# prashantpandeygit/solvingpapers

Measured on AMD Instinct MI355X. Metric: training tokens/sec, LLaMA3-8B-shape bf16, higher is better.
Workload: dtype bf16; 1 GPU; model=llama3_8b, global_batch=4, seq_len=8192, parallelism=dp1, micro_batch=1, grad_accum=4, params=8030261248

## Files before the change

### csrc/include/attn_params.h

```cpp
#pragma once
#include "attn_common.h"

#define SPA_DBG_BRH(b, r, R, h, H) (SPA_DBG_OK(b, p.B) & SPA_DBG_OK(r, R) & SPA_DBG_OK(h, H))

namespace spa {

struct AttnParams {
  const bf16* q; const bf16* k; const bf16* v; const bf16* o; const bf16* dout;
  bf16* out; bf16* dq; bf16* dk; bf16* dv;
  float* lse; const float* lse_in; float* delta; float* dqacc;
  int B, H, Hkv, Tq, Tk;
  long sqb, sqt, sqh, skb, skt, skh, svb, svt, svh, sob, sot, soh;
  long sdob, sdot, sdoh;
  long sdqb, sdqt, sdqh, sdkb, sdkt, sdkh, sdvb, sdvt, sdvh;
  float scale;
  float scale_log2;
  int causal_off;
  int hsplit;
  float* dkacc; float* dvacc;
  unsigned seed_lo, seed_hi, drop_thr;
  float drop_scale;
  const int64_t* seed_ptr;
  long long* stamp;
  int xcd;
  bf16* dsbuf;
  long ds_kvstride;
  int ds_nqt, ds_nkt;
  int ksplit;
  float* part;
  float* mlpart;
  int part_ld;
  int vhalf;
  float* rowk;
  int rowk_ld;
};

void launch_dkdv5(AttnParams& p, bool causal, hipStream_t st);
void launch_bwd_short(AttnParams& p, bool causal, hipStream_t st);

__device__ __forceinline__ long ds_index(int qt, int kt, int g, int G, int nkt, bool causal) {
  const int qb = qt >> 1, t = qt & 1;
  const long step = causal ? (long)qb * (qb + 1) + kt : (long)qb * nkt + kt;
  return (step * G + g) * 2 + t;
}
inline long ds_kv_elems(int nq64, int nkt, int G, bool causal) {
  return 1024L * 2 * G * (causal ? (long)nq64 * (nq64 + 1) : (long)nq64 * nkt);
}
__device__ __forceinline__ int ds_slot(int s, int h, int k) { return (k >> 2) * 16 + (2 * s + h) * 4 + (k & 3); }

template <int HD, int NDT = HD / 32>
__device__ __forceinline__ void store_kv_grad(const AttnParams& p, const f32x16 (&acc)[NDT], bool is_k,
                                              int b, int hk, int key, int split, int hh, int dt0 = 0) {
  if (key >= p.Tk) return;
  if (!(SPA_DBG_BRH(b, key, p.Tk, hk, p.Hkv) & SPA_DBG_OK(split, p.hsplit))) return;
  static_assert(NDT <= HD / 32, "store_kv_grad: more tiles than the head dim");
  constexpr int DT = NDT;
  if (p.hsplit == 1) {
    bf16* dst = (is_k ? p.dk + b * p.sdkb + (long)key * p.sdkt + hk * p.sdkh
                      : p.dv + b * p.sdvb + (long)key * p.sdvt + hk * p.sdvh) + 32 * dt0;
    const float sc = is_k ? p.scale : 1.f;
#pragma unroll
    for (int dt = 0; dt < DT; ++dt)
#pragma unroll
      for (int g = 0; g < 4; ++g) {
        bf16x4 w;
#pragma unroll
        for (int i = 0; i < 4; ++i) w[i] = (bf16)(acc[dt][4 * g + i] * sc);
        *reinterpret_cast<bf16x4*>(dst + 32 * dt + 8 * g + 4 * hh) = w;
      }
  } else {
    float* dst = (is_k ? p.dkacc : p.dvacc) +
                 ((((long)split * p.B + b) * p.Tk + key) * p.Hkv + hk) * HD + 32 * dt0;
#pragma unroll
    for (int dt = 0; dt < DT; ++dt)
#pragma unroll
      for (int g = 0; g < 4; ++g) {
        f32x4 w;
#pragma unroll
        for (int i = 0; i < 4; ++i) w[i] = acc[dt][4 * g + i];
        *reinterpret_cast<f32x4*>(dst + 32 * dt + 8 * g + 4 * hh) = w;
      }
  }
// ... 5 lines not shown
```

### csrc/kernels/attention.hip

```cpp
#include "attn_common.h"
#include "attn_params.h"

SPA_DEBUG_TU("attention.hip")

namespace spa {



__device__ __forceinline__ unsigned mix32(unsigned x) {
  x ^= x >> 16; x *= 0x7feb352dU; x ^= x >> 15; x *= 0x846ca68bU; x ^= x >> 16;
  return x;
}
__device__ __forceinline__ unsigned drop_base(const AttnParams& p, int b, int h) {
  unsigned lo = p.seed_lo, hi = p.seed_hi;
  if (p.seed_ptr) {
    const uint64_t sd = (uint64_t)*p.seed_ptr;
    lo = (unsigned)(sd & 0xffffffffu);
    hi = (unsigned)(sd >> 32);
  }
  return mix32(lo ^ mix32(hi + (unsigned)(b * p.H + h) * 0x9E3779B9U));
}
__device__ __forceinline__ bool drop_keep(unsigned base, int q, int key, unsigned thr) {
  return (mix32(base + (unsigned)q * 0x85EBCA6BU + (unsigned)key * 0xC2B2AE35U) >> 8) >= thr;
}
// ... 15 lines not shown
  } else {
    const int nbh = p.H * p.B;
    const int bh = bi % nbh;
    qb = bi / nbh;
    if (causal) qb = nqb - 1 - qb;
    h = bh % p.H;
    b = bh / p.H;
  }
}

template <int HDK, int HDV> constexpr int attn_bn() { return (HDK >= 256 || HDV >= 256) ? 32 : 64; }

#ifndef FWD_PV_SCHED
#define FWD_PV_SCHED 1
#endif
template <int HDK, int HDV, int NW, bool CAUSAL, bool DROP>
__global__ __launch_bounds__(NW * 64) void attn_fwd_kernel(AttnParams p) {
  constexpr int BN = attn_bn<HDK, HDV>(), NSUB = BN / 32, BM = 32 * NW, KS = HDK / 16, DT = HDV / 32;
  constexpr int NT = NW * 64, IK = img_w<HDK>(), IV = img_w<HDV>();
  constexpr int TK = BN * IK, TV = BN * IV, TB = TK + TV;
  __shared__ __attribute__((aligned(16))) bf16 smem[2 * TB];
  const int tid = threadIdx.x, lane = tid & 63, wave = tid >> 6;
  const int lq = lane & 31, hh = lane >> 5;
  const int nqb = cdiv(p.Tq, BM);
  const int si = blockIdx.x % p.ksplit;
  int qb, b, h;
  q_block_map(p, nqb, CAUSAL, qb, b, h, blockIdx.x / p.ksplit, gridDim.x / p.ksplit);
  const int hk = h / (p.H / p.Hkv);
  SPA_DBG_CHECK(qb, nqb);
  SPA_DBG_CHECK(hk, p.Hkv);
  (void)SPA_DBG_BRH(b, 0, 1, h, p.H);
  const int q0 = __builtin_amdgcn_readfirstlane(qb * BM + wave * 32);
  const int q = q0 + lq;
  const float c = p.scale_log2;
  const int vcol = blockIdx.y * p.vhalf;
  unsigned dbase = 0;
  if constexpr (DROP) dbase = drop_base(p, b, h);

  bf16x8 qf[KS];
  {
    const bf16* qp = p.q + b * p.sqb + (long)q * p.sqt + h * p.sqh + 8 * hh;
#pragma unroll
    for (int s = 0; s < KS; ++s) qf[s] = q < p.Tq ? *reinterpret_cast<const bf16x8*>(qp + 16 * s) : zero8();
  }
  f32x16 o[DT];
#pragma unroll
  for (int i = 0; i < DT; ++i) o[i] = splat16(0.f);
  float m = -1e30f, l = 0.f;

  int kend = p.Tk;
  if (CAUSAL) kend = min(p.Tk, qb * BM + BM + p.causal_off);
  const int wave_kend = q0 >= p.Tq ? 0 : CAUSAL ? min(p.Tk, q0 + 32 + p.causal_off) : p.Tk;
  const int ntiles_all = kend > 0 ? cdiv(kend, BN) : 0;
  const int kper = cdiv(ntiles_all, p.ksplit);
  const int jbeg = min(ntiles_all, si * kper);
  const int ntiles = min(ntiles_all, jbeg + kper) - jbeg;
  const int kb0 = jbeg * BN;

// ... 1108 lines not shown
      store_kv_grad<HDV>(p, av, false, b, hk, key, split, hh);
    }
  }
#if SPA_DKDV3_STAMP
  DK3_TICK(4);
  if (p.stamp != nullptr && lane < 8) {
    long long v = 0;
#pragma unroll
    for (int i = 0; i < 5; ++i) v = lane == i ? seg[i] : v;
    v = lane == 5 ? (long long)(total + 1) : lane == 6 ? ts_ - t_start : v;
    p.stamp[((long)blockIdx.x * 8 + wave) * 8 + lane] = v;
  }
#endif
}

template <int HD, bool CAUSAL, bool NT>
__global__ __launch_bounds__(256, 2) void attn_bwd_dq_ds_kernel(AttnParams p) {
  static_assert(HD == 128, "dq_ds: head dim 128 (K tile = 4 KiB-row images of 256 B)");
  constexpr int DT = HD / 32, KIMG = 32 * HD, WSLOT = 2 * 1024, SLOT = KIMG + 4 * WSLOT, NSLOT = 3;
  __shared__ __attribute__((aligned(16))) bf16 smem[NSLOT * SLOT];
  const int tid = threadIdx.x, lane = tid & 63;
  const int wave = __builtin_amdgcn_readfirstlane(tid >> 6);
  const int hh = lane >> 5;
  const int G = p.H / p.Hkv;
  const int nq64 = cdiv(p.Tq, 64);
  const int upkv = nq64 * G;
  const int wgpkv = cdiv(upkv, 4);
  const int nbkv = p.B * p.Hkv;
  const int bkv = blockIdx.x % nbkv;
  const int w = CAUSAL ? wgpkv - 1 - (int)(blockIdx.x / nbkv) : (int)(blockIdx.x / nbkv);
  const int b = bkv / p.Hkv, hk = bkv % p.Hkv;
// ... 84 lines not shown
        if (jj + 1 < nsteps) asm volatile("s_waitcnt vmcnt(6)" ::: "memory");
        else asm volatile("s_waitcnt vmcnt(0)" ::: "memory");
        asm volatile("s_waitcnt lgkmcnt(0)" ::: "memory");
        __builtin_amdgcn_s_barrier();
        if (jj + 2 < nsteps) issue(jj + 2, (r + 2) % 3);
        compute(jj, smem + r * SLOT);
      }
    }
  }
  if (!uvalid) return;
#pragma unroll
  for (int t = 0; t < 2; ++t) {
    const int q = qb * 64 + 32 * t + (lane & 31);
    if (q >= p.Tq || !SPA_DBG_BRH(b, q, p.Tq, h, p.H)) continue;
    bf16* op = p.dq + b * p.sdqb + (long)q * p.sdqt + h * p.sdqh;
#pragma unroll
    for (int dt = 0; dt < DT; ++dt)
#pragma unroll
      for (int g = 0; g < 4; ++g) {
        bf16x4 wv;
#pragma unroll
        for (int i = 0; i < 4; ++i) wv[i] = (bf16)(acc[t][dt][4 * g + i] * p.scale);
        *reinterpret_cast<bf16x4*>(op + 32 * dt + 8 * g + 4 * hh) = wv;
      }
  }
}

template <int HDK, bool CAUSAL, bool NT>
__global__ __launch_bounds__(256, 2) void attn_bwd_dq_ds256_kernel(AttnParams p) {
  static_assert(HDK == 256 || HDK == 192, "dq_ds256: q/k head dim 192 or 256");
  constexpr int HD = 256, DT = HDK / 32, KIMG = 32 * HD, WSLOT = 1024, SLOT = KIMG + 4 * WSLOT, NSLOT = 3;
  __shared__ __attribute__((aligned(16))) bf16 smem[NSLOT * SLOT];
  const int tid = threadIdx.x, lane = tid & 63;
  const int wave = __builtin_amdgcn_readfirstlane(tid >> 6);
  const int hh = lane >> 5;
  const int G = p.H / p.Hkv;
  const int nqt = cdiv(p.Tq, 32);
  const int upkv = nqt * G;
  const int wgpkv = cdiv(upkv, 4);
// ... 296 lines not shown
  TORCH_CHECK(dropout_p >= 0.0 && dropout_p < 1.0, "attention dropout p must be in [0, 1)");
  p.seed_lo = (unsigned)(seed & 0xffffffffu);
  p.seed_hi = (unsigned)(((uint64_t)seed >> 32) & 0xffffffffu);
  p.drop_thr = (unsigned)std::llround(dropout_p * 16777216.0);
  p.drop_scale = (float)(1.0 / (1.0 - dropout_p));
}

static int attn_ksplit(long blocks, int ntk) {
  const char* e = getenv("SPA_ATTN_KSPLIT");
  if (e) return std::max(1, std::min(atoi(e), std::max(1, ntk)));
  int ks = 1;
  while (blocks * ks < 512 && ks < 8 && ntk / (2 * ks) >= 4) ks *= 2;
  return ks;
}

std::vector<at::Tensor> attn_fwd(const at::Tensor& q, const at::Tensor& k, const at::Tensor& v, double scale,
                                 bool causal, double dropout_p, int64_t seed,
                                 const c10::optional<at::Tensor>& seed_t) {
  check_qkv(q, "q"); check_qkv(k, "k"); check_qkv(v, "v");
  const int B = q.size(0), Tq = q.size(1), H = q.size(2), HDK = q.size(3), HDV = v.size(3);
  const int Tk = k.size(1), Hkv = k.size(2);
  TORCH_CHECK(k.size(0) == B && v.size(0) == B && v.size(1) == Tk && v.size(2) == Hkv && k.size(3) == HDK,
              "attn: shape mismatch");
  TORCH_CHECK(H % Hkv == 0, "attn: H must be a multiple of Hkv");
  const bool drop = dropout_p > 0.0;
  TORCH_CHECK(!drop || HDK == HDV, "attn: dropout needs equal q/k and v head dims");
  DeviceGuard g(q.device());
  auto out = at::empty({B, Tq, H, HDV}, q.options());
  auto lse = at::empty({B, H, Tq}, q.options().dtype(at::kFloat));
  AttnParams p{};
  p.q = (const bf16*)q.data_ptr(); p.k = (const bf16*)k.data_ptr(); p.v = (const bf16*)v.data_ptr();
  p.out = (bf16*)out.data_ptr(); p.lse = lse.data_ptr<float>();
  p.B = B; p.H = H; p.Hkv = Hkv; p.Tq = Tq; p.Tk = Tk;
  fill_strides(p, q, k, v);
  fill_dropout(p, dropout_p, seed, seed_t);
  p.sob = out.stride(0); p.sot = out.stride(1); p.soh = out.stride(2);
  p.scale = (float)scale; p.scale_log2 = (float)(scale * 1.4426950408889634);
  p.causal_off = Tk - Tq;
  p.hsplit = 1;
  p.ksplit = 1;
  p.xcd = xcd_order(B, Hkv);
  if (B * Tq * H == 0) return {out, lse};
  auto st = stream();
  const char* f2e = getenv("SPA_ATTN_FWD256");
  const bool pshare = !(f2e && atoi(f2e) == 0) && HDK == 256 && HDV == 256 && !drop;
  const char* sve = getenv("SPA_ATTN_SPLITV");
  const bool splitv = !pshare && !(sve && atoi(sve) == 0) && HDK == 256 && HDV == 256 && !drop;
  const int nw = splitv || pshare ? 8 : (HDK <= 192 && HDV <= 192) || (HDK == 256 && HDV == 128) ? 8 : 4;
  const int blocks = cdiv(Tq, pshare ? 128 : 32 * nw) * H * B * (splitv ? 2 : 1);
  const int ntk = cdiv(Tk, (HDK >= 256 || HDV >= 256) ? 32 : 64);
  p.ksplit = attn_ksplit(blocks, ntk);
  at::Tensor part;
  if (p.ksplit > 1) {
    const long rows = (long)B * H * Tq;
    part = at::empty({(long)p.ksplit * rows * (HDV + 2)}, q.options().dtype(at::kFloat));
    p.part = part.data_ptr<float>();
    p.part_ld = HDV;
    p.mlpart = p.part + (long)p.ksplit * rows * HDV;
  }
  const int gx = blocks / (splitv ? 2 : 1) * p.ksplit;
  if (pshare) {
    if (causal) attn_fwd256p_kernel<true><<<gx, 512, 0, st>>>(p);
    else attn_fwd256p_kernel<false><<<gx, 512, 0, st>>>(p);
  } else if (splitv) {
    p.vhalf = 128;
    if (causal) attn_fwd_kernel<256, 128, 8, true, false><<<dim3(gx, 2), 512, 0, st>>>(p);
    else attn_fwd_kernel<256, 128, 8, false, false><<<dim3(gx, 2), 512, 0, st>>>(p);
  } else {
    HDKV_SWITCH(HDK, HDV, {
      constexpr int NW = fwd_waves<HDK_, HDV_>();
      constexpr bool SQ = HDK_ == HDV_;
      if (drop) {
        if constexpr (SQ) {
          if (causal) attn_fwd_kernel<HDK_, HDV_, NW, true, true><<<gx, NW * 64, 0, st>>>(p);
          else attn_fwd_kernel<HDK_, HDV_, NW, false, true><<<gx, NW * 64, 0, st>>>(p);
        }
      } else {
        if (causal) attn_fwd_kernel<HDK_, HDV_, NW, true, false><<<gx, NW * 64, 0, st>>>(p);
        else attn_fwd_kernel<HDK_, HDV_, NW, false, false><<<gx, NW * 64, 0, st>>>(p);
      }
    });
  }
  if (p.ksplit > 1) {
    const long n = (long)B * H * Tq * (HDV / 8);
    HDKV_SWITCH(HDK, HDV, { attn_fwd_merge_kernel<HDV_><<<(int)cdiv(n, 256L), 256, 0, st>>>(p); });
  }
  SPA_LAUNCH_CHECK();
  return {out, lse};
}

template <int HDK, int HDV, bool DROP>
static void launch_bwd(AttnParams& p, bool causal, bool fused, int dkdv_mode, int nkv, hipStream_t st,
                       const at::TensorOptions& bf16_opts) {
// ... 9 lines not shown
      else attn_bwd_dkdv_kernel<HDK, HDV, false, MT, true, false><<<g2, 256, 0, st>>>(p);
      const long n = rows * (HDK / 8);
      attn_dq_store_kernel<HDK><<<(int)std::min<long>((n + 255) / 256, 65536), 256, 0, st>>>(p);
      return;
    }
  }
  if constexpr (HDK == 128 && HDV == 128 && !DROP) {
    const char* de = getenv("SPA_ATTN_DQ_DS");
    const bool want = !(de && atoi(de) == 0);
    const long kv_bytes = 2 * ds_kv_elems(cdiv(p.Tq, 64), cdiv(p.Tk, 32), p.H / p.Hkv, causal);
    if (want && p.hsplit == 1 && p.Tk > 0 && dkdv_mode == 0 && (!causal || p.causal_off == 0) &&
        kv_bytes < 0x7fffffffL) {
      const long rows = (long)p.B * p.Tq * p.H;
      const char* v5e = getenv("SPA_ATTN_DKDV5");
      const bool v5 = !(v5e && atoi(v5e) == 0);
      if (!v5) attn_delta_kernel<HDK><<<(int)cdiv(rows, 256 / (HDK / 8)), 256, 0, st>>>(p);
      p.ds_nqt = cdiv(p.Tq, 32);
      p.ds_nkt = cdiv(p.Tk, 32);
      p.ds_kvstride = ds_kv_elems(cdiv(p.Tq, 64), p.ds_nkt, p.H / p.Hkv, causal);
      at::Tensor dsb = at::empty({(long)p.B * p.Hkv * p.ds_kvstride}, bf16_opts);
      p.dsbuf = (bf16*)dsb.data_ptr();
      at::Tensor rowk;
      if (v5) {
        p.rowk_ld = cdiv(p.Tq, 64) * 64;
        rowk = at::empty({(long)p.B * p.H * 2 * p.rowk_ld}, bf16_opts.dtype(at::kFloat));
        p.rowk = rowk.data_ptr<float>();
        launch_dkdv5(p, causal, st);
      } else if (causal) attn_bwd_dkdv3_kernel<HDK, HDV, true, true><<<nkv, 512, 0, st>>>(p);
      else attn_bwd_dkdv3_kernel<HDK, HDV, false, true><<<nkv, 512, 0, st>>>(p);
      const int G = p.H / p.Hkv;
      const int wg = cdiv(cdiv(p.Tq, 64) * G, 4) * p.B * p.Hkv;
      const char* ne = getenv("SPA_ATTN_DS_NT");
      const bool nt = !(ne && atoi(ne) == 0);
      if (nt) {
        if (causal) attn_bwd_dq_ds_kernel<HDK, true, true><<<wg, 256, 0, st>>>(p);
        else attn_bwd_dq_ds_kernel<HDK, false, true><<<wg, 256, 0, st>>>(p);
      } else {
        if (causal) attn_bwd_dq_ds_kernel<HDK, true, false><<<wg, 256, 0, st>>>(p);
        else attn_bwd_dq_ds_kernel<HDK, false, false><<<wg, 256, 0, st>>>(p);
      }
      return;
    }
  }
  if constexpr (((HDK == 256 && HDV == 256) || (HDK == 192 && HDV == 128)) && !DROP) {
    const char* de = getenv("SPA_ATTN_DQ_DS");
    const int dsm = de ? atoi(de) : 1;
    const bool want = dsm != 0;
    const int G = p.H / p.Hkv;
    const long kv_bytes = 2 * ds_kv_elems(cdiv(p.Tq, 64), cdiv(p.Tk, 32), G, causal);
// ... 90 lines not shown
    const long rows = (long)p.B * p.Tk * p.Hkv;
    attn_kv_reduce_kernel<HDK><<<(int)std::min<long>((rows * (HDK / 8) + 255) / 256, 65536), 256, 0, st>>>(p, 1);
    attn_kv_reduce_kernel<HDV><<<(int)std::min<long>((rows * (HDV / 8) + 255) / 256, 65536), 256, 0, st>>>(p, 0);
  }
}

static at::Tensor& last_stamps() {
  static at::Tensor t;
  return t;
}
at::Tensor attn_bwd_stamps() { return last_stamps().defined() ? last_stamps().view({-1, 8}).clone() : at::Tensor(); }

void attn_bwd(const at::Tensor& dout, const at::Tensor& q, const at::Tensor& k, const at::Tensor& v,
              const at::Tensor& out, const at::Tensor& lse, const at::Tensor& dq, const at::Tensor& dk,
              const at::Tensor& dv, double scale, bool causal, double dropout_p, int64_t seed,
              const c10::optional<at::Tensor>& seed_t) {
  check_qkv(dout, "dout"); check_qkv(q, "q"); check_qkv(k, "k"); check_qkv(v, "v"); check_qkv(out, "out");
  check_qkv(dq, "dq"); check_qkv(dk, "dk"); check_qkv(dv, "dv");
  const int B = q.size(0), Tq = q.size(1), H = q.size(2), HDK = q.size(3), HDV = v.size(3);
  const int Tk = k.size(1), Hkv = k.size(2);
  TORCH_CHECK(lse.is_contiguous() && lse.numel() == (int64_t)B * H * Tq);
  TORCH_CHECK(dq.sizes() == q.sizes() && dk.sizes() == k.sizes() && dv.sizes() == v.sizes());
  TORCH_CHECK(dout.sizes() == out.sizes() && out.size(3) == HDV && out.size(2) == H && out.size(1) == Tq);
  const bool drop = dropout_p > 0.0;
  TORCH_CHECK(!drop || HDK == HDV, "attn: dropout needs equal q/k and v head dims");
  DeviceGuard g(q.device());
  auto delta = at::empty({B, H, Tq}, q.options().dtype(at::kFloat));
  AttnParams p{};
  p.q = (const bf16*)q.data_ptr(); p.k = (const bf16*)k.data_ptr(); p.v = (const bf16*)v.data_ptr();
  p.o = (const bf16*)out.data_ptr(); p.dout = (const bf16*)dout.data_ptr();
  p.dq = (bf16*)dq.data_ptr(); p.dk = (bf16*)dk.data_ptr(); p.dv = (bf16*)dv.data_ptr();
  p.lse_in = lse.data_ptr<float>(); p.delta = delta.data_ptr<float>();
  p.B = B; p.H = H; p.Hkv = Hkv; p.Tq = Tq; p.Tk = Tk;
  fill_strides(p, q, k, v);
  fill_dropout(p, dropout_p, seed, seed_t);
  p.sob = out.stride(0); p.sot = out.stride(1); p.soh = out.stride(2);
  p.sdob = dout.stride(0); p.sdot = dout.stride(1); p.sdoh = dout.stride(2);
  p.sdqb = dq.stride(0); p.sdqt = dq.stride(1); p.sdqh = dq.stride(2);
  p.sdkb = dk.stride(0); p.sdkt = dk.stride(1); p.sdkh = dk.stride(2);
  p.sdvb = dv.stride(0); p.sdvt = dv.stride(1); p.sdvh = dv.stride(2);
  p.scale = (float)scale; p.scale_log2 = (float)(scale * 1.4426950408889634);
  p.causal_off = Tk - Tq;
  p.xcd = xcd_order(B, Hkv);
  p.ksplit = 1;
  if (B * H == 0) return;
  auto st = stream();
  if (Tq == 0) { dk.zero_(); dv.zero_(); return; }
  static const bool want_fused = getenv("SPA_ATTN_BWD_FUSED") && atoi(getenv("SPA_ATTN_BWD_FUSED")) != 0;
  const bool fused = want_fused && Tk > 0 && HDK <= 128 && HDK == HDV && !drop;
  const char* sse = getenv("SPA_ATTN_SHORT");
  const bool want_short = !(sse && atoi(sse) == 0);
  if (want_short && !fused && !drop && HDK == 64 && HDV == 64 && H == Hkv && Tq <= 256 && Tk <= 256) {
    launch_bwd_short(p, causal, st);
    SPA_LAUNCH_CHECK();
    return;
  }
  at::Tensor dqacc;
  if (fused) {
    dqacc = at::zeros({B, Tq, H, HDK}, q.options().dtype(at::kFloat));
    p.dqacc = dqacc.data_ptr<float>();
  }
  const int dkdv_mode = getenv("SPA_ATTN_DKDV") ? atoi(getenv("SPA_ATTN_DKDV")) : 0;
  const int G = H / Hkv;
  const int nkv = cdiv(Tk, 128) * Hkv * B;
  int hsplit = 1;
  const char* kbe = getenv("SPA_ATTN_KVBLOCKS");
  const int kvblocks = kbe ? std::max(1, atoi(kbe)) : 512;
  if (!fused)
    while (nkv * hsplit < kvblocks && hsplit < G) {
// ... 16 lines not shown
  }
  at::Tensor kvacc;
  if (hsplit > 1) {
    kvacc = at::empty({(long)hsplit * B * Tk * Hkv * (HDK + HDV)}, q.options().dtype(at::kFloat));
    p.dkacc = kvacc.data_ptr<float>();
    p.dvacc = p.dkacc + (long)hsplit * B * Tk * Hkv * HDK;
  }
  HDKV_SWITCH(HDK, HDV, {
    if (drop) {
      if constexpr (HDK_ == HDV_) launch_bwd<HDK_, HDV_, true>(p, causal, false, dkdv_mode, nkv, st, q.options());
    } else {
      launch_bwd<HDK_, HDV_, false>(p, causal, fused, dkdv_mode, nkv, st, q.options());
    }
  });
  SPA_LAUNCH_CHECK();
}

}

TORCH_LIBRARY_FRAGMENT(spa, m) {
  m.def("attn_fwd(Tensor q, Tensor k, Tensor v, float scale, bool causal, float dropout_p=0.0, int seed=0, "
        "Tensor? seed_t=None) -> Tensor[]");
  m.def("attn_bwd(Tensor dout, Tensor q, Tensor k, Tensor v, Tensor out, Tensor lse, Tensor(a!) dq, Tensor(b!) dk, "
        "Tensor(c!) dv, float scale, bool causal, float dropout_p=0.0, int seed=0, Tensor? seed_t=None) -> ()");
  m.def("attn_bwd_stamps() -> Tensor", &spa::attn_bwd_stamps);
}
TORCH_LIBRARY_IMPL(spa, CUDA, m) {
  m.impl("attn_fwd", &spa::attn_fwd);
  m.impl("attn_bwd", &spa::attn_bwd);
}
```

### csrc/kernels/attention_dkdv5.hip

```cpp
#include "attn_common.h"
#include "attn_params.h"

SPA_DEBUG_TU("attention_dkdv5.hip")

namespace spa {

__device__ __forceinline__ void dma4_asm(__amdgpu_buffer_rsrc_t rs, unsigned voff, unsigned lds) {
  unsigned keep;
  asm volatile("s_mov_b32 %0, m0\n\ts_mov_b32 m0, %3\n\ts_nop 0\n\tbuffer_load_dword %1, %2, 0 offen lds\n\ts_mov_b32 m0, %0"
               : "=&s"(keep) : "v"(voff), "s"(rs), "s"(lds) : "memory");
}

template <int HD>
__global__ __launch_bounds__(256) void attn_rowk_kernel(AttnParams p) {
  constexpr int TPR = HD / 8, RPB = 256 / TPR;
  const int Tqp = p.rowk_ld;
  const long row = (long)blockIdx.x * RPB + threadIdx.x / TPR;
  const int t = threadIdx.x % TPR;
  const long nrows = (long)p.B * Tqp * p.H;
  float acc = 0.f;
  long b = 0, q = 0, h = 0;
  if (row < nrows) {
    h = row % p.H;
    q = (row / p.H) % Tqp;
// ... 25 lines not shown
    const long long tn_ = (long long)__builtin_amdgcn_s_memtime();    \
    seg[i] += tn_ - ts_;                                              \
    ts_ = tn_;                                                        \
  } while (0)
#else
#define D5_TICK(i) \
  do {             \
  } while (0)
#endif

struct D5Tile {
  int g, qi;
  long qoff, doff, roff;
};

template <bool CAUSAL>
__global__ __launch_bounds__(512) void attn_bwd_dkdv5_kernel(AttnParams p) {
  constexpr int HD = 128, MT = 2, BMQ = 64, BNK = 128, KS = HD / 16, DT = HD / 32;
  constexpr int TQ = BMQ * HD, TB = 2 * TQ, PSLOT = 4 * MT * 2 * 64 * 8, RSF = 2 * BMQ;
  __shared__ __attribute__((aligned(16))) bf16 smem[3 * TB + 2 * PSLOT + 3 * RSF * 2];
  bf16* const pimg = smem + 3 * TB;
  float* const rowc = reinterpret_cast<float*>(pimg + 2 * PSLOT);
  const int tid = threadIdx.x, lane = tid & 63;
  const int wave = __builtin_amdgcn_readfirstlane(tid >> 6);
  const int pair = wave & 3, role = wave >> 2;
  const int hh = lane >> 5;
  const int nbh = p.Hkv * p.B;
  const int bh = blockIdx.x % nbh;
  const int kb = blockIdx.x / nbh;
  const int hk = bh % p.Hkv, b = bh / p.Hkv;
  SPA_DBG_CHECK(b, p.B);
// ... 220 lines not shown
  };
  if (total == 0) {
  } else if (role == 0) {
    for (int k = 0; k <= total; k += 3) {
      interval(k, IC<0>{}, IC<0>{});
      interval(k + 1, IC<1>{}, IC<0>{});
      interval(k + 2, IC<2>{}, IC<0>{});
    }
  } else {
    for (int k = 0; k <= total; k += 3) {
      interval(k, IC<0>{}, IC<1>{});
      interval(k + 1, IC<1>{}, IC<1>{});
      interval(k + 2, IC<2>{}, IC<1>{});
    }
  }
  store_kv_grad<HD>(p, acc, role == 1, b, hk, key, 0, hh);
#if SPA_DKDV5_STAMP
  D5_TICK(4);
  if (p.stamp != nullptr && lane < 8) {
    long long v = 0;
#pragma unroll
    for (int i = 0; i < 5; ++i) v = lane == i ? seg[i] : v;
    v = lane == 5 ? (long long)(total + 1) : lane == 6 ? ts_ - t_start : v;
    p.stamp[((long)blockIdx.x * 8 + wave) * 8 + lane] = v;
  }
#endif
}

void launch_dkdv5(AttnParams& p, bool causal, hipStream_t st) {
  const long rows = (long)p.B * p.rowk_ld * p.H;
  attn_rowk_kernel<128><<<(int)cdiv(rows, 256 / 16), 256, 0, st>>>(p);
  const int nkv = cdiv(p.Tk, 128) * p.Hkv * p.B;
  if (causal) attn_bwd_dkdv5_kernel<true><<<nkv, 512, 0, st>>>(p);
  else attn_bwd_dkdv5_kernel<false><<<nkv, 512, 0, st>>>(p);
}

}
```

### csrc/kernels/rope.hip

```cpp
#include "spa_common.h"
#include "fp8_quant.h"
#include "paged_kv.h"
#include <type_traits>

SPA_DEBUG_TU("rope.hip")

namespace spa {

template <typename DT, int MODE>
__global__ __launch_bounds__(256) void rope_kernel(DT* __restrict__ x, const float* __restrict__ cosT,
                                                   const float* __restrict__ sinT, const int* __restrict__ pos,
                                                   long sb, long st, long sh, int B, int T, int nrot, int hd,
                                                   int pos_off, float sign) {
  const int vpr = hd / 8;
  const long total = (long)B * T * nrot * vpr;
  for (long i = blockIdx.x * 256L + threadIdx.x; i < total; i += (long)gridDim.x * 256) {
    const int v = i % vpr;
    long r = i / vpr;
    const int hh = r % nrot;
    r /= nrot;
    const int t = r % T;
    const int b = r / T;
    const int ps = pos ? pos[b * T + t] : t + pos_off;
    DT* p = x + b * sb + t * st + hh * sh;
    const float* c = cosT + (long)ps * (hd / 2);
    const float* s = sinT + (long)ps * (hd / 2);
    if constexpr (MODE == 0 || MODE == 2) {
      float a[8];
      load8(p + v * 8, a);
      const f32x4 cv = *reinterpret_cast<const f32x4*>(c + v * 4);
      const f32x4 sv = *reinterpret_cast<const f32x4*>(s + v * 4);
#pragma unroll
      for (int k = 0; k < 4; ++k) {
        const float x0 = a[2 * k], x1 = a[2 * k + 1];
        const float cs = cv[k];
        if constexpr (MODE == 0) {
          const float sn = sign * sv[k];
          a[2 * k] = x0 * cs - x1 * sn;
          a[2 * k + 1] = x0 * sn + x1 * cs;
        } else if (sign > 0.f) {
          a[2 * k] = cs * (x0 + x1);
          a[2 * k + 1] = sv[k] * (x1 - x0);
        } else {
          a[2 * k] = cs * x0 - sv[k] * x1;
          a[2 * k + 1] = cs * x0 + sv[k] * x1;
        }
      }
      store8(p + v * 8, a);
    } else {
      if (v >= vpr / 2) continue;
      float a[8], bq[8];
      load8(p + v * 8, a);
      load8(p + hd / 2 + v * 8, bq);
      float cv[8], sv[8];
// ... 445 lines not shown
```

### solvingpapers_amd/models/llama3.py

```python
from __future__ import annotations

import math
from dataclasses import dataclass, field, replace
from typing import List, Optional

import torch
import torch.nn as nn

from ..infer.cache import new_kv_cache
from ..infer.graph import DecodeState, ExtendState
from ..infer.sampling import sample
from ..ops import attention_packed, embedding, linear, linear_cross_entropy, rms_norm, rope_packed_
from ..ops.linear import swiglu_mlp
from ..ops.attention import kv_cache_attend, kv_cache_write, rope_kv_cache_write_
from ..ops.layout import gather_rows
from ..ops.rope import RopeCache, apply_rope
from ..utils.grad import mark_ready


@dataclass
class LlamaConfig:
    vocab_size: int = 50257
    dim: int = 256
    n_layers: int = 2
    n_heads: int = 4
    n_kv_heads: int = 2
    ffn_hidden: int = 1024
# ... 63 lines not shown
            H, KV = c.n_heads, c.n_kv_heads
            x4 = qkv.view(B, T, H + 2 * KV, hd)
            cos, sin = RopeCache.get(pos.max_len, hd, c.rope_theta, qkv.device, c.ref_freqs)
            rope_kv_cache_write_(kv_cache, x4, cos, sin, pos.positions, pos.index, H, KV, 0, per_row=pos.per_row)
            o = kv_cache_attend(x4[:, :, :H], kv_cache, causal=True, kv_len=pos.kv_len, per_row=pos.per_row)
            return linear(o.reshape(B, T, H * hd), self.wo)
        if kv_cache is None and self.cp_group is not None:
            import torch.distributed as dist
            from ..parallel.context_parallel import context_parallel_attention
            H, KV = c.n_heads, c.n_kv_heads
            off = dist.get_rank(self.cp_group) * T
            qkv = rope_packed_(qkv, H + KV, c.rope_theta, off, head_dim=hd, ref_freqs=c.ref_freqs)
            x4 = qkv.view(B, T, H + 2 * KV, hd)
            o = context_parallel_attention(x4[:, :, :H], x4[:, :, H:H + KV], x4[:, :, H + KV:], self.cp_group)
        elif kv_cache is None:
            qkv = rope_packed_(qkv, c.n_heads + c.n_kv_heads, c.rope_theta, 0, head_dim=hd, ref_freqs=c.ref_freqs)
            o = attention_packed(qkv, c.n_heads, c.n_kv_heads, causal=True, head_dim=hd)
        else:
            qkv = qkv.view(B, T, c.n_heads + 2 * c.n_kv_heads, hd)
            q = apply_rope(qkv[:, :, :c.n_heads], c.rope_theta, pos, ref_freqs=c.ref_freqs)
            k = apply_rope(qkv[:, :, c.n_heads:c.n_heads + c.n_kv_heads], c.rope_theta, pos, ref_freqs=c.ref_freqs)
            v = qkv[:, :, c.n_heads + c.n_kv_heads:]
            kv_cache_write(kv_cache, k, v, pos)
            o = kv_cache_attend(q, kv_cache, pos + T, causal=True, fresh=(k, v) if pos == 0 else None)
        return linear(o.reshape(B, T, c.n_heads * hd), self.wo)

    def forward(self, res, delta, kv_cache=None, pos=0):
        c = self.c
        if res is None:
            n1 = rms_norm(delta, self.attention_norm, c.norm_eps)
            h = delta
        else:
# ... 160 lines not shown
```

### solvingpapers_amd/ops/__init__.py

```python
from . import _ext, reference
from .activation import act, elu, geglu, gelu, glu, leaky_relu, prelu, relu, sigmoid, silu, swiglu
from .attention import (KV8, attention_packed, decode_attention, flash_attention, kv_cache_attend, kv_cache_write,
                        rope_kv_cache_write_)
from .embedding import embedding
from .linear import Linear, linear
from .moe import MoEPlan, combine, gather, grouped_gemm, grouped_linear, moe_ffn, permute, route
from .norm import layer_norm, rms_norm
from .rope import apply_rope, rope_packed_
from .sampling import sample_logits, u01
from .xent import cross_entropy, linear_cross_entropy, per_row_loss

__all__ = [
    "act", "elu", "geglu", "gelu", "glu", "leaky_relu", "prelu", "relu", "sigmoid", "silu", "swiglu",
    "KV8", "kv_cache_attend", "kv_cache_write", "rope_kv_cache_write_",
    "attention_packed", "decode_attention", "flash_attention", "embedding", "Linear", "linear", "layer_norm", "rms_norm",
    "apply_rope", "rope_packed_", "MoEPlan", "combine", "gather", "grouped_gemm", "grouped_linear", "moe_ffn",
    "permute", "route", "cross_entropy", "linear_cross_entropy", "per_row_loss", "reference", "sample_logits", "u01",
]
```

### solvingpapers_amd/ops/attention.py

```python
from __future__ import annotations

import math

import os

import torch

from . import _ext, reference

FLASH_PAIRS = ((64, 64), (128, 128), (256, 256), (192, 128))
FLASH_HD = (64, 128, 256)


def _pair_for(dqk, dv):
    best = None
    for a, b in FLASH_PAIRS:
        if a >= dqk and b >= dv and (best is None or a + b < best[0] + best[1]):
            best = (a, b)
    return best


def _flash_ok(q):
    return q.is_cuda and q.dtype == torch.bfloat16 and (q.dim() == 3 or q.shape[-1] in FLASH_HD)

# ... 65 lines not shown
        ctx.dropout_p, ctx.seed = dropout_p, seed
        return torch.ops.aten._unsafe_view(out, (B, T, H * hd))

    @staticmethod
    def backward(ctx, dout):
        qkv, out, lse = ctx.saved_tensors
        H, Hkv, hd = ctx.H, ctx.Hkv, ctx.hd
        B, T = qkv.shape[0], qkv.shape[1]
        dqkv = torch.empty_like(qkv)
        x4 = qkv.view(B, T, H + 2 * Hkv, hd)
        d4 = dqkv.view(B, T, H + 2 * Hkv, hd)
        _ext.ops().attn_bwd(dout.contiguous().view(B, T, H, hd), x4[:, :, :H], x4[:, :, H:H + Hkv],
                            x4[:, :, H + Hkv:], out, lse, d4[:, :, :H], d4[:, :, H:H + Hkv], d4[:, :, H + Hkv:],
                            ctx.scale, ctx.causal, ctx.dropout_p, *_seed_args(ctx.seed))
        return dqkv, None, None, None, None, None, None, None


FLASH_F32_HD = (16, 32, 64, 128, 256)


class _FlashF32Fn(torch.autograd.Function):

    @staticmethod
    def forward(ctx, q, k, v, causal, scale, dropout_p, seed):
        si, st = _seed_args(seed)
        out, lse = _ext.ops().attn_f32_fwd(q, k, v, scale, causal, dropout_p, si, st)
        ctx.save_for_backward(q, k, v, out, lse)
        ctx.causal, ctx.scale, ctx.dropout_p, ctx.seed = causal, scale, dropout_p, seed
        return out

# ... 454 lines not shown
```

Baseline: 22640 tokens/s.

## Fuse RoPE into flash attention forward Q load and backward dQ/dK stores

```diff
diff --git a/csrc/include/attn_params.h b/csrc/include/attn_params.h
--- a/csrc/include/attn_params.h
+++ b/csrc/include/attn_params.h
@@ -1,5 +1,6 @@
 #pragma once
 #include "attn_common.h"
+#include "rope_pair.h"
 
 #define SPA_DBG_BRH(b, r, R, h, H) (SPA_DBG_OK(b, p.B) & SPA_DBG_OK(r, R) & SPA_DBG_OK(h, H))
 
@@ -33,9 +34,15 @@
   int vhalf;
   float* rowk;
   int rowk_ld;
+  const float* rope_cos; const float* rope_sin;
+  int rope_off;
+  float rope_sign;
+  int rope, rope_done;
 };
 
 void launch_dkdv5(AttnParams& p, bool causal, hipStream_t st);
+void rope_(const at::Tensor& x, const at::Tensor& cos, const at::Tensor& sin, const c10::optional<at::Tensor>& pos,
+           int64_t nrot, int64_t pos_off, int64_t mode, bool inverse);
 void launch_bwd_short(AttnParams& p, bool causal, hipStream_t st);
 
 __device__ __forceinline__ long ds_index(int qt, int kt, int g, int G, int nkt, bool causal) {
@@ -48,7 +55,26 @@
 }
 __device__ __forceinline__ int ds_slot(int s, int h, int k) { return (k >> 2) * 16 + (2 * s + h) * 4 + (k & 3); }
 
-template <int HD, int NDT = HD / 32>
+__device__ __forceinline__ void rope_bf16x4(bf16x4& w, const f32x2 cv, const f32x2 sv, const float sign) {
+  float a[4];
+#pragma unroll
+  for (int i = 0; i < 4; ++i) a[i] = (float)w[i];
+#pragma unroll
+  for (int k = 0; k < 2; ++k) rope_pair(a[2 * k], a[2 * k + 1], cv[k], sv[k], sign);
+#pragma unroll
+  for (int i = 0; i < 4; ++i) w[i] = (bf16)a[i];
+}
+__device__ __forceinline__ void rope_bf16x8(bf16x8& w, const f32x4 cv, const f32x4 sv, const float sign) {
+  float a[8];
+#pragma unroll
+  for (int i = 0; i < 8; ++i) a[i] = (float)w[i];
+#pragma unroll
+  for (int k = 0; k < 4; ++k) rope_pair(a[2 * k], a[2 * k + 1], cv[k], sv[k], sign);
+#pragma unroll
+  for (int i = 0; i < 8; ++i) w[i] = (bf16)a[i];
+}
+
+template <int HD, int NDT = HD / 32, bool ROPE = false>
 __device__ __forceinline__ void store_kv_grad(const AttnParams& p, const f32x16 (&acc)[NDT], bool is_k,
                                               int b, int hk, int key, int split, int hh, int dt0 = 0) {
   if (key >= p.Tk) return;
@@ -59,6 +85,19 @@
     bf16* dst = (is_k ? p.dk + b * p.sdkb + (long)key * p.sdkt + hk * p.sdkh
                       : p.dv + b * p.sdvb + (long)key * p.sdvt + hk * p.sdvh) + 32 * dt0;
     const float sc = is_k ? p.scale : 1.f;
+    f32x2 cv[DT][4], sv[DT][4];
+    if constexpr (ROPE) {
+      if (is_k) {
+        const long tr = ((long)p.rope_off + key) * (HD / 2) + 16 * dt0 + 2 * hh;
+#pragma unroll
+        for (int dt = 0; dt < DT; ++dt)
+#pragma unroll
+          for (int g = 0; g < 4; ++g) {
+            cv[dt][g] = *reinterpret_cast<const f32x2*>(p.rope_cos + tr + 16 * dt + 4 * g);
+            sv[dt][g] = *reinterpret_cast<const f32x2*>(p.rope_sin + tr + 16 * dt + 4 * g);
+          }
+      }
+    }
 #pragma unroll
     for (int dt = 0; dt < DT; ++dt)
 #pragma unroll
@@ -66,6 +105,9 @@
         bf16x4 w;
 #pragma unroll
         for (int i = 0; i < 4; ++i) w[i] = (bf16)(acc[dt][4 * g + i] * sc);
+        if constexpr (ROPE) {
+          if (is_k) rope_bf16x4(w, cv[dt][g], sv[dt][g], p.rope_sign);
+        }
         *reinterpret_cast<bf16x4*>(dst + 32 * dt + 8 * g + 4 * hh) = w;
       }
   } else {
diff --git a/csrc/include/rope_pair.h b/csrc/include/rope_pair.h
--- /dev/null
+++ b/csrc/include/rope_pair.h
@@ -0,0 +1,12 @@
+#pragma once
+
+namespace spa {
+
+__device__ __forceinline__ void rope_pair(float& x0r, float& x1r, const float cs, const float sv, const float sign) {
+  const float x0 = x0r, x1 = x1r;
+  const float sn = sign * sv;
+  x0r = __builtin_fmaf(cs, x0, -(sn * x1));
+  x1r = __builtin_fmaf(cs, x1, sn * x0);
+}
+
+}
diff --git a/csrc/kernels/attention.hip b/csrc/kernels/attention.hip
--- a/csrc/kernels/attention.hip
+++ b/csrc/kernels/attention.hip
@@ -53,8 +53,9 @@
 #ifndef FWD_PV_SCHED
 #define FWD_PV_SCHED 1
 #endif
-template <int HDK, int HDV, int NW, bool CAUSAL, bool DROP>
+template <int HDK, int HDV, int NW, bool CAUSAL, bool DROP, bool ROPE = false>
 __global__ __launch_bounds__(NW * 64) void attn_fwd_kernel(AttnParams p) {
+  static_assert(!ROPE || (HDK == 128 && HDV == 128 && !DROP), "fused RoPE: head dim 128 without dropout");
   constexpr int BN = attn_bn<HDK, HDV>(), NSUB = BN / 32, BM = 32 * NW, KS = HDK / 16, DT = HDV / 32;
   constexpr int NT = NW * 64, IK = img_w<HDK>(), IV = img_w<HDV>();
   constexpr int TK = BN * IK, TV = BN * IV, TB = TK + TV;
@@ -81,6 +82,22 @@
     const bf16* qp = p.q + b * p.sqb + (long)q * p.sqt + h * p.sqh + 8 * hh;
 #pragma unroll
     for (int s = 0; s < KS; ++s) qf[s] = q < p.Tq ? *reinterpret_cast<const bf16x8*>(qp + 16 * s) : zero8();
+    if constexpr (ROPE) {
+      if (q < p.Tq && SPA_DBG_BRH(b, q, p.Tq, h, p.H)) {
+        const long tr = ((long)p.rope_off + q) * (HDK / 2) + 4 * hh;
+        f32x4 cv[KS], sv[KS];
+#pragma unroll
+        for (int s = 0; s < KS; ++s) {
+          cv[s] = *reinterpret_cast<const f32x4*>(p.rope_cos + tr + 8 * s);
+          sv[s] = *reinterpret_cast<const f32x4*>(p.rope_sin + tr + 8 * s);
+        }
+#pragma unroll
+        for (int s = 0; s < KS; ++s) rope_bf16x8(qf[s], cv[s], sv[s], p.rope_sign);
+        bf16* qw = const_cast<bf16*>(qp);
+#pragma unroll
+        for (int s = 0; s < KS; ++s) *reinterpret_cast<bf16x8*>(qw + 16 * s) = qf[s];
+      }
+    }
   }
   f32x16 o[DT];
 #pragma unroll
@@ -1219,7 +1236,7 @@
 #endif
 }
 
-template <int HD, bool CAUSAL, bool NT>
+template <int HD, bool CAUSAL, bool NT, bool ROPE = false>
 __global__ __launch_bounds__(256, 2) void attn_bwd_dq_ds_kernel(AttnParams p) {
   static_assert(HD == 128, "dq_ds: head dim 128 (K tile = 4 KiB-row images of 256 B)");
   constexpr int DT = HD / 32, KIMG = 32 * HD, WSLOT = 2 * 1024, SLOT = KIMG + 4 * WSLOT, NSLOT = 3;
@@ -1334,15 +1351,31 @@
     const int q = qb * 64 + 32 * t + (lane & 31);
     if (q >= p.Tq || !SPA_DBG_BRH(b, q, p.Tq, h, p.H)) continue;
     bf16* op = p.dq + b * p.sdqb + (long)q * p.sdqt + h * p.sdqh;
-#pragma unroll
-    for (int dt = 0; dt < DT; ++dt)
-#pragma unroll
-      for (int g = 0; g < 4; ++g) {
-        bf16x4 wv;
-#pragma unroll
-        for (int i = 0; i < 4; ++i) wv[i] = (bf16)(acc[t][dt][4 * g + i] * p.scale);
-        *reinterpret_cast<bf16x4*>(op + 32 * dt + 8 * g + 4 * hh) = wv;
-      }
+    const long tr = ROPE ? ((long)p.rope_off + q) * (HD / 2) + 2 * hh : 0;
+#pragma unroll
+    for (int dp = 0; dp < DT; dp += 2) {
+      f32x2 cv[2][4], sv[2][4];
+      if constexpr (ROPE) {
+#pragma unroll
+        for (int d = 0; d < 2; ++d)
+#pragma unroll
+          for (int g = 0; g < 4; ++g) {
+            cv[d][g] = *reinterpret_cast<const f32x2*>(p.rope_cos + tr + 16 * (dp + d) + 4 * g);
+            sv[d][g] = *reinterpret_cast<const f32x2*>(p.rope_sin + tr + 16 * (dp + d) + 4 * g);
+          }
+      }
+#pragma unroll
+      for (int d = 0; d < 2; ++d)
+#pragma unroll
+        for (int g = 0; g < 4; ++g) {
+          const int dt = dp + d;
+          bf16x4 wv;
+#pragma unroll
+          for (int i = 0; i < 4; ++i) wv[i] = (bf16)(acc[t][dt][4 * g + i] * p.scale);
+          if constexpr (ROPE) rope_bf16x4(wv, cv[d][g], sv[d][g], p.rope_sign);
+          *reinterpret_cast<bf16x4*>(op + 32 * dt + 8 * g + 4 * hh) = wv;
+        }
+    }
   }
 }
 
@@ -1669,9 +1702,46 @@
   return ks;
 }
 
+static void check_rope(const at::Tensor& q, const at::Tensor& k, const at::Tensor& cos,
+                       const c10::optional<at::Tensor>& sin, int64_t rope_off) {
+  TORCH_CHECK(sin.has_value(), "attn rope: rope_cos and rope_sin come together");
+  TORCH_CHECK(q.size(1) == k.size(1), "attn rope: q and k must hold the same tokens (Tq == Tk)");
+  for (const at::Tensor* t : {&cos, &*sin})
+    TORCH_CHECK(t->is_cuda() && t->device() == q.device() && t->scalar_type() == at::kFloat && t->dim() == 2 &&
+                    t->is_contiguous() && t->size(1) == q.size(3) / 2 && (uintptr_t)t->data_ptr() % 16 == 0,
+                "attn rope: fp32 [Tmax, hd/2] tables on q's device");
+  TORCH_CHECK(sin->size(0) == cos.size(0) && rope_off >= 0 && rope_off + q.size(1) <= cos.size(0) &&
+                  rope_off + q.size(1) < (1L << 31),
+              "attn rope: table too short");
+}
+
+static void rope_qk_(const at::Tensor& q, const at::Tensor& k, const at::Tensor& cos, const at::Tensor& sin,
+                     int64_t rope_off, bool inverse, bool do_q, bool do_k) {
+  const int64_t H = q.size(2), Hkv = k.size(2);
+  const bool packed = q.strides() == k.strides() && q.size(0) == k.size(0) && q.size(1) == k.size(1) &&
+                      (const bf16*)k.data_ptr() == (const bf16*)q.data_ptr() + H * q.stride(2);
+  if (do_q && do_k && packed) {
+    rope_(q.as_strided({q.size(0), q.size(1), H + Hkv, q.size(3)}, q.strides()), cos, sin, c10::nullopt, H + Hkv,
+          rope_off, 0, inverse);
+    return;
+  }
+  if (do_q) rope_(q, cos, sin, c10::nullopt, H, rope_off, 0, inverse);
+  if (do_k) rope_(k, cos, sin, c10::nullopt, Hkv, rope_off, 0, inverse);
+}
+
+static void fill_rope(AttnParams& p, const at::Tensor& cos, const at::Tensor& sin, int64_t rope_off, float sign) {
+  p.rope = 1;
+  p.rope_cos = cos.data_ptr<float>();
+  p.rope_sin = sin.data_ptr<float>();
+  p.rope_off = (int)rope_off;
+  p.rope_sign = sign;
+}
+
 std::vector<at::Tensor> attn_fwd(const at::Tensor& q, const at::Tensor& k, const at::Tensor& v, double scale,
                                  bool causal, double dropout_p, int64_t seed,
-                                 const c10::optional<at::Tensor>& seed_t) {
+                                 const c10::optional<at::Tensor>& seed_t,
+                                 const c10::optional<at::Tensor>& rope_cos,
+                                 const c10::optional<at::Tensor>& rope_sin, int64_t rope_off) {
   check_qkv(q, "q"); check_qkv(k, "k"); check_qkv(v, "v");
   const int B = q.size(0), Tq = q.size(1), H = q.size(2), HDK = q.size(3), HDV = v.size(3);
   const int Tk = k.size(1), Hkv = k.size(2);
@@ -1680,6 +1750,8 @@
   TORCH_CHECK(H % Hkv == 0, "attn: H must be a multiple of Hkv");
   const bool drop = dropout_p > 0.0;
   TORCH_CHECK(!drop || HDK == HDV, "attn: dropout needs equal q/k and v head dims");
+  const bool rope = rope_cos.has_value();
+  if (rope) check_rope(q, k, *rope_cos, rope_sin, rope_off);
   DeviceGuard g(q.device());
   auto out = at::empty({B, Tq, H, HDV}, q.options());
   auto lse = at::empty({B, H, Tq}, q.options().dtype(at::kFloat));
@@ -1695,7 +1767,10 @@
   p.hsplit = 1;
   p.ksplit = 1;
   p.xcd = xcd_order(B, Hkv);
-  if (B * Tq * H == 0) return {out, lse};
+  if (B * Tq * H == 0) {
+    if (rope) rope_qk_(q, k, *rope_cos, *rope_sin, rope_off, false, true, true);
+    return {out, lse};
+  }
   auto st = stream();
   const char* f2e = getenv("SPA_ATTN_FWD256");
   const bool pshare = !(f2e && atoi(f2e) == 0) && HDK == 256 && HDV == 256 && !drop;
@@ -1714,6 +1789,11 @@
     p.mlpart = p.part + (long)p.ksplit * rows * HDV;
   }
   const int gx = blocks / (splitv ? 2 : 1) * p.ksplit;
+  if (rope) {
+    const bool fuse_q = HDK == 128 && HDV == 128 && !drop && p.ksplit == 1;
+    rope_qk_(q, k, *rope_cos, *rope_sin, rope_off, false, !fuse_q, true);
+    if (fuse_q) fill_rope(p, *rope_cos, *rope_sin, rope_off, 1.f);
+  }
   if (pshare) {
     if (causal) attn_fwd256p_kernel<true><<<gx, 512, 0, st>>>(p);
     else attn_fwd256p_kernel<false><<<gx, 512, 0, st>>>(p);
@@ -1731,7 +1811,13 @@
           else attn_fwd_kernel<HDK_, HDV_, NW, false, true><<<gx, NW * 64, 0, st>>>(p);
         }
       } else {
-        if (causal) attn_fwd_kernel<HDK_, HDV_, NW, true, false><<<gx, NW * 64, 0, st>>>(p);
+        constexpr bool RP = HDK_ == 128 && HDV_ == 128;
+        if (RP && p.rope) {
+          if constexpr (RP) {
+            if (causal) attn_fwd_kernel<HDK_, HDV_, NW, true, false, true><<<gx, NW * 64, 0, st>>>(p);
+            else attn_fwd_kernel<HDK_, HDV_, NW, false, false, true><<<gx, NW * 64, 0, st>>>(p);
+          }
+        } else if (causal) attn_fwd_kernel<HDK_, HDV_, NW, true, false><<<gx, NW * 64, 0, st>>>(p);
         else attn_fwd_kernel<HDK_, HDV_, NW, false, false><<<gx, NW * 64, 0, st>>>(p);
       }
     });
@@ -1771,6 +1857,8 @@
       const long rows = (long)p.B * p.Tq * p.H;
       const char* v5e = getenv("SPA_ATTN_DKDV5");
       const bool v5 = !(v5e && atoi(v5e) == 0);
+      p.rope = p.rope && v5;
+      p.rope_done = p.rope;
       if (!v5) attn_delta_kernel<HDK><<<(int)cdiv(rows, 256 / (HDK / 8)), 256, 0, st>>>(p);
       p.ds_nqt = cdiv(p.Tq, 32);
       p.ds_nkt = cdiv(p.Tk, 32);
@@ -1789,7 +1877,15 @@
       const int wg = cdiv(cdiv(p.Tq, 64) * G, 4) * p.B * p.Hkv;
       const char* ne = getenv("SPA_ATTN_DS_NT");
       const bool nt = !(ne && atoi(ne) == 0);
-      if (nt) {
+      if (p.rope) {
+        if (nt) {
+          if (causal) attn_bwd_dq_ds_kernel<HDK, true, true, true><<<wg, 256, 0, st>>>(p);
+          else attn_bwd_dq_ds_kernel<HDK, false, true, true><<<wg, 256, 0, st>>>(p);
+        } else {
+          if (causal) attn_bwd_dq_ds_kernel<HDK, true, false, true><<<wg, 256, 0, st>>>(p);
+          else attn_bwd_dq_ds_kernel<HDK, false, false, true><<<wg, 256, 0, st>>>(p);
+        }
+      } else if (nt) {
         if (causal) attn_bwd_dq_ds_kernel<HDK, true, true><<<wg, 256, 0, st>>>(p);
         else attn_bwd_dq_ds_kernel<HDK, false, true><<<wg, 256, 0, st>>>(p);
       } else {
@@ -1910,7 +2006,8 @@
 void attn_bwd(const at::Tensor& dout, const at::Tensor& q, const at::Tensor& k, const at::Tensor& v,
               const at::Tensor& out, const at::Tensor& lse, const at::Tensor& dq, const at::Tensor& dk,
               const at::Tensor& dv, double scale, bool causal, double dropout_p, int64_t seed,
-              const c10::optional<at::Tensor>& seed_t) {
+              const c10::optional<at::Tensor>& seed_t, const c10::optional<at::Tensor>& rope_cos,
+              const c10::optional<at::Tensor>& rope_sin, int64_t rope_off) {
   check_qkv(dout, "dout"); check_qkv(q, "q"); check_qkv(k, "k"); check_qkv(v, "v"); check_qkv(out, "out");
   check_qkv(dq, "dq"); check_qkv(dk, "dk"); check_qkv(dv, "dv");
   const int B = q.size(0), Tq = q.size(1), H = q.size(2), HDK = q.size(3), HDV = v.size(3);
@@ -1939,6 +2036,11 @@
   p.causal_off = Tk - Tq;
   p.xcd = xcd_order(B, Hkv);
   p.ksplit = 1;
+  const bool rope = rope_cos.has_value();
+  if (rope) {
+    check_rope(q, k, *rope_cos, rope_sin, rope_off);
+    fill_rope(p, *rope_cos, *rope_sin, rope_off, -1.f);
+  }
   if (B * H == 0) return;
   auto st = stream();
   if (Tq == 0) { dk.zero_(); dv.zero_(); return; }
@@ -1949,6 +2051,7 @@
   if (want_short && !fused && !drop && HDK == 64 && HDV == 64 && H == Hkv && Tq <= 256 && Tk <= 256) {
     launch_bwd_short(p, causal, st);
     SPA_LAUNCH_CHECK();
+    if (rope) rope_qk_(dq, dk, *rope_cos, *rope_sin, rope_off, true, true, true);
     return;
   }
   at::Tensor dqacc;
@@ -1995,15 +2098,17 @@
     }
   });
   SPA_LAUNCH_CHECK();
+  if (rope && !p.rope_done) rope_qk_(dq, dk, *rope_cos, *rope_sin, rope_off, true, true, true);
 }
 
 }
 
 TORCH_LIBRARY_FRAGMENT(spa, m) {
-  m.def("attn_fwd(Tensor q, Tensor k, Tensor v, float scale, bool causal, float dropout_p=0.0, int seed=0, "
-        "Tensor? seed_t=None) -> Tensor[]");
+  m.def("attn_fwd(Tensor(a!) q, Tensor(b!) k, Tensor v, float scale, bool causal, float dropout_p=0.0, int seed=0, "
+        "Tensor? seed_t=None, Tensor? rope_cos=None, Tensor? rope_sin=None, int rope_off=0) -> Tensor[]");
   m.def("attn_bwd(Tensor dout, Tensor q, Tensor k, Tensor v, Tensor out, Tensor lse, Tensor(a!) dq, Tensor(b!) dk, "
-        "Tensor(c!) dv, float scale, bool causal, float dropout_p=0.0, int seed=0, Tensor? seed_t=None) -> ()");
+        "Tensor(c!) dv, float scale, bool causal, float dropout_p=0.0, int seed=0, Tensor? seed_t=None, "
+        "Tensor? rope_cos=None, Tensor? rope_sin=None, int rope_off=0) -> ()");
   m.def("attn_bwd_stamps() -> Tensor", &spa::attn_bwd_stamps);
 }
 TORCH_LIBRARY_IMPL(spa, CUDA, m) {
diff --git a/csrc/kernels/attention_dkdv5.hip b/csrc/kernels/attention_dkdv5.hip
--- a/csrc/kernels/attention_dkdv5.hip
+++ b/csrc/kernels/attention_dkdv5.hip
@@ -63,7 +63,7 @@
   long qoff, doff, roff;
 };
 
-template <bool CAUSAL>
+template <bool CAUSAL, bool ROPE = false>
 __global__ __launch_bounds__(512) void attn_bwd_dkdv5_kernel(AttnParams p) {
   constexpr int HD = 128, MT = 2, BMQ = 64, BNK = 128, KS = HD / 16, DT = HD / 32;
   constexpr int TQ = BMQ * HD, TB = 2 * TQ, PSLOT = 4 * MT * 2 * 64 * 8, RSF = 2 * BMQ;
@@ -314,7 +314,7 @@
       interval(k + 2, IC<2>{}, IC<1>{});
     }
   }
-  store_kv_grad<HD>(p, acc, role == 1, b, hk, key, 0, hh);
+  store_kv_grad<HD, DT, ROPE>(p, acc, role == 1, b, hk, key, 0, hh);
 #if SPA_DKDV5_STAMP
   D5_TICK(4);
   if (p.stamp != nullptr && lane < 8) {
@@ -331,7 +331,10 @@
   const long rows = (long)p.B * p.rowk_ld * p.H;
   attn_rowk_kernel<128><<<(int)cdiv(rows, 256 / 16), 256, 0, st>>>(p);
   const int nkv = cdiv(p.Tk, 128) * p.Hkv * p.B;
-  if (causal) attn_bwd_dkdv5_kernel<true><<<nkv, 512, 0, st>>>(p);
+  if (p.rope) {
+    if (causal) attn_bwd_dkdv5_kernel<true, true><<<nkv, 512, 0, st>>>(p);
+    else attn_bwd_dkdv5_kernel<false, true><<<nkv, 512, 0, st>>>(p);
+  } else if (causal) attn_bwd_dkdv5_kernel<true><<<nkv, 512, 0, st>>>(p);
   else attn_bwd_dkdv5_kernel<false><<<nkv, 512, 0, st>>>(p);
 }
 
diff --git a/csrc/kernels/rope.hip b/csrc/kernels/rope.hip
--- a/csrc/kernels/rope.hip
+++ b/csrc/kernels/rope.hip
@@ -1,6 +1,7 @@
 #include "spa_common.h"
 #include "fp8_quant.h"
 #include "paged_kv.h"
+#include "rope_pair.h"
 #include <type_traits>
 
 SPA_DEBUG_TU("rope.hip")
@@ -35,9 +36,7 @@
         const float x0 = a[2 * k], x1 = a[2 * k + 1];
         const float cs = cv[k];
         if constexpr (MODE == 0) {
-          const float sn = sign * sv[k];
-          a[2 * k] = x0 * cs - x1 * sn;
-          a[2 * k + 1] = x0 * sn + x1 * cs;
+          rope_pair(a[2 * k], a[2 * k + 1], cs, sv[k], sign);
         } else if (sign > 0.f) {
           a[2 * k] = cs * (x0 + x1);
           a[2 * k + 1] = sv[k] * (x1 - x0);
diff --git a/solvingpapers_amd/models/llama3.py b/solvingpapers_amd/models/llama3.py
--- a/solvingpapers_amd/models/llama3.py
+++ b/solvingpapers_amd/models/llama3.py
@@ -10,7 +10,7 @@
 from ..infer.cache import new_kv_cache
 from ..infer.graph import DecodeState, ExtendState
 from ..infer.sampling import sample
-from ..ops import attention_packed, embedding, linear, linear_cross_entropy, rms_norm, rope_packed_
+from ..ops import attention_packed_rope, embedding, linear, linear_cross_entropy, rms_norm, rope_packed_
 from ..ops.linear import swiglu_mlp
 from ..ops.attention import kv_cache_attend, kv_cache_write, rope_kv_cache_write_
 from ..ops.layout import gather_rows
@@ -104,8 +104,8 @@
             x4 = qkv.view(B, T, H + 2 * KV, hd)
             o = context_parallel_attention(x4[:, :, :H], x4[:, :, H:H + KV], x4[:, :, H + KV:], self.cp_group)
         elif kv_cache is None:
-            qkv = rope_packed_(qkv, c.n_heads + c.n_kv_heads, c.rope_theta, 0, head_dim=hd, ref_freqs=c.ref_freqs)
-            o = attention_packed(qkv, c.n_heads, c.n_kv_heads, causal=True, head_dim=hd)
+            o = attention_packed_rope(qkv, c.n_heads, c.n_kv_heads, c.rope_theta, 0, causal=True, head_dim=hd,
+                                      ref_freqs=c.ref_freqs)
         else:
             qkv = qkv.view(B, T, c.n_heads + 2 * c.n_kv_heads, hd)
             q = apply_rope(qkv[:, :, :c.n_heads], c.rope_theta, pos, ref_freqs=c.ref_freqs)
diff --git a/solvingpapers_amd/ops/__init__.py b/solvingpapers_amd/ops/__init__.py
--- a/solvingpapers_amd/ops/__init__.py
+++ b/solvingpapers_amd/ops/__init__.py
@@ -1,7 +1,7 @@
 from . import _ext, reference
 from .activation import act, elu, geglu, gelu, glu, leaky_relu, prelu, relu, sigmoid, silu, swiglu
-from .attention import (KV8, attention_packed, decode_attention, flash_attention, kv_cache_attend, kv_cache_write,
-                        rope_kv_cache_write_)
+from .attention import (KV8, attention_packed, attention_packed_rope, decode_attention, flash_attention, kv_cache_attend,
+                        kv_cache_write, rope_kv_cache_write_)
 from .embedding import embedding
 from .linear import Linear, linear
 from .moe import MoEPlan, combine, gather, grouped_gemm, grouped_linear, moe_ffn, permute, route
@@ -13,7 +13,8 @@
 __all__ = [
     "act", "elu", "geglu", "gelu", "glu", "leaky_relu", "prelu", "relu", "sigmoid", "silu", "swiglu",
     "KV8", "kv_cache_attend", "kv_cache_write", "rope_kv_cache_write_",
-    "attention_packed", "decode_attention", "flash_attention", "embedding", "Linear", "linear", "layer_norm", "rms_norm",
+    "attention_packed", "attention_packed_rope", "decode_attention", "flash_attention", "embedding", "Linear", "linear",
+    "layer_norm", "rms_norm",
     "apply_rope", "rope_packed_", "MoEPlan", "combine", "gather", "grouped_gemm", "grouped_linear", "moe_ffn",
     "permute", "route", "cross_entropy", "linear_cross_entropy", "per_row_loss", "reference", "sample_logits", "u01",
 ]
diff --git a/solvingpapers_amd/ops/attention.py b/solvingpapers_amd/ops/attention.py
--- a/solvingpapers_amd/ops/attention.py
+++ b/solvingpapers_amd/ops/attention.py
@@ -103,6 +103,54 @@
                             x4[:, :, H + Hkv:], out, lse, d4[:, :, :H], d4[:, :, H:H + Hkv], d4[:, :, H + Hkv:],
                             ctx.scale, ctx.causal, ctx.dropout_p, *_seed_args(ctx.seed))
         return dqkv, None, None, None, None, None, None, None
+
+
+class _PackedRopeFn(torch.autograd.Function):
+
+    @staticmethod
+    def forward(ctx, qkv, H, Hkv, hd, causal, scale, cos, sin, pos_off):
+        B, T = qkv.shape[0], qkv.shape[1]
+        x4 = qkv.view(B, T, H + 2 * Hkv, hd)
+        q, k, v = x4[:, :, :H], x4[:, :, H:H + Hkv], x4[:, :, H + Hkv:]
+        out, lse = _ext.ops().attn_fwd(q, k, v, scale, causal, 0.0, 0, None, cos, sin, pos_off)
+        ctx.mark_dirty(qkv)
+        ctx.set_materialize_grads(False)
+        ctx.save_for_backward(qkv, out, lse, cos, sin)
+        ctx.H, ctx.Hkv, ctx.hd, ctx.causal, ctx.scale, ctx.pos_off = H, Hkv, hd, causal, scale, pos_off
+        return torch.ops.aten._unsafe_view(out, (B, T, H * hd)), qkv
+
+    @staticmethod
+    def backward(ctx, dout, dqkv_out):
+        qkv, out, lse, cos, sin = ctx.saved_tensors
+        H, Hkv, hd = ctx.H, ctx.Hkv, ctx.hd
+        B, T = qkv.shape[0], qkv.shape[1]
+        assert dqkv_out is None, "attention_packed_rope: the rotated qkv buffer has no gradient path"
+        if dout is None:
+            return (None,) * 9
+        dqkv = torch.empty_like(qkv)
+        x4 = qkv.view(B, T, H + 2 * Hkv, hd)
+        d4 = dqkv.view(B, T, H + 2 * Hkv, hd)
+        _ext.ops().attn_bwd(dout.contiguous().view(B, T, H, hd), x4[:, :, :H], x4[:, :, H:H + Hkv],
+                            x4[:, :, H + Hkv:], out, lse, d4[:, :, :H], d4[:, :, H:H + Hkv], d4[:, :, H + Hkv:],
+                            ctx.scale, ctx.causal, 0.0, 0, None, cos, sin, ctx.pos_off)
+        return dqkv, None, None, None, None, None, None, None, None
+
+
+def _attn_rope_on():
+    return os.environ.get("SPA_ATTN_ROPE", "1") != "0"
+
+
+def attention_packed_rope(qkv, H, Hkv, theta=10000.0, pos_off=0, causal=True, scale=None, head_dim=None,
+                          ref_freqs=False):
+    from .rope import RopeCache, rope_packed_
+    hd = head_dim if head_dim is not None else qkv.shape[-1]
+    if qkv.is_cuda and qkv.dtype == torch.bfloat16 and hd in FLASH_HD and _attn_rope_on():
+        T = qkv.shape[1]
+        scale = float(scale) if scale is not None else 1.0 / math.sqrt(hd)
+        cos, sin = RopeCache.get(pos_off + T, hd, theta, qkv.device, ref_freqs)
+        return _PackedRopeFn.apply(qkv, H, Hkv, hd, causal, scale, cos, sin, int(pos_off))[0]
+    qkv = rope_packed_(qkv, H + Hkv, theta, pos_off, head_dim=hd, ref_freqs=ref_freqs)
+    return attention_packed(qkv, H, Hkv, causal=causal, scale=scale, head_dim=hd)
 
 
 FLASH_F32_HD = (16, 32, 64, 128, 256)
```

New measurement: 22660 tokens/s (median of 2 runs). About the same (+0.1%).
